# synsense/HaghighatshoarMuir2024

Hardware: AMD Instinct MI355X
Metric: audio samples/sec through STHT+RZCC+SNN beamform, 7-mic 48kHz 360-DoA; DoA MAE vs ref (higher is better)
Workload: dtype f64

## Files before the change

### __graft_entry__.py

```python
import os
import subprocess
import sys

ROOT = os.path.dirname(os.path.abspath(__file__))
if ROOT not in sys.path:
    sys.path.insert(0, ROOT)


def build() -> None:
    env = dict(os.environ)
    subprocess.check_call(["make", "-s", "-j4", "-C", os.path.join(ROOT, "haghighatshoarmuir2024_amd", "csrc")], env=env)
    subprocess.check_call(["make", "-s", "-C", os.path.join(ROOT, "oracle"), "_build/libmicloc_oracle.so", "_build/libmicloc_oracle_asan.so"], env=env)
    subprocess.check_call([sys.executable, os.path.join(ROOT, "tools", "dev", "make_variant.py"), "stht_valu", "stht_one_tile", "ws_k4", "ws_sparse_lif"], env=env)
    import haghighatshoarmuir2024_amd
    from haghighatshoarmuir2024_amd import _lib

    lib = _lib.load()
    assert lib.micloc_abi_version() == 1


def smoke() -> None:
    import numpy as np
    import torch

    from haghighatshoarmuir2024_amd.runtime import Plan
    from oracle import oracle as O

    assert torch.cuda.is_available(), "smoke() needs the MI355X"
    torch.cuda.set_device(0)
    fs, M, G, T, B = 48_000, 7, 64, 2400, 4
    rng = np.random.RandomState(0)
    ker = O.stht_kernel(fs, 10e-3)
    b, a = O.bandpass(fs, [1000.0, 2000.0])
    w = O.robust_width(fs, 2000.0)
    tau = 1 / (2 * np.pi * 2000.0)
    nir = O.neuron_kernel(np.arange(T) / fs, [tau, tau])
    W = rng.randn(2 * M, G)
    W /= np.linalg.norm(W, axis=0, keepdims=True)
    t = np.arange(T) / fs
    x = np.sin(2 * np.pi * 1500 * t)[None, :, None] * np.ones((B, 1, M)) + 0.5 * rng.randn(B, T, M)
    plan = Plan(M, ker, b, a, w, True, device="cuda:0")
    plan.set_neuron_kernel(nir)
    plan.set_bf_mat(W)
    out = plan.snn_pipeline(plan.to_device(x), want_spikes=True, want_power=True)
    torch.cuda.synchronize()
    spikes = out["spikes"].cpu().numpy()
    power = out["power"].cpu().numpy()
    argmax = out["argmax"].cpu().numpy()
    for i in range(B):
        ref = O.snn_chain(x[i], ker, b, a, w, True, nir, W, want=("spikes", "power"))
        assert np.array_equal(spikes[i], ref["spikes"]), "spikes differ from the oracle"
        assert np.allclose(power[i], ref["power"], rtol=1e-12, atol=0), "power differs from the oracle"
        assert int(argmax[i]) == ref["argmax"]
    print(f"smoke ok: {B} trials x {T} frames, {int((spikes != 0).sum())} spikes bit-exact, power rel err <= 1e-12")


if __name__ == "__main__":
    cmd = sys.argv[1] if len(sys.argv) > 1 else "build"
    {"build": build, "smoke": smoke}[cmd]()
```

### haghighatshoarmuir2024_amd/csrc/beamform.hip

```cpp
#include "micloc_internal.h"

namespace micloc {

typedef double double4_t __attribute__((ext_vector_type(4)));
typedef double double2_t __attribute__((ext_vector_type(2)));

constexpr int BF_THREADS = BF_WAVES * 64;

typedef unsigned uint2_t __attribute__((ext_vector_type(2)));

__device__ __forceinline__ double row_sum4(double x)
{
    unsigned lo = __double2loint(x), hi = __double2hiint(x);
    uint2_t a = __builtin_amdgcn_permlane16_swap(lo, lo, false, false);
    uint2_t b = __builtin_amdgcn_permlane16_swap(hi, hi, false, false);
    const double s = __hiloint2double(b[0], a[0]) + __hiloint2double(b[1], a[1]);
    lo = __double2loint(s);
    hi = __double2hiint(s);
    a = __builtin_amdgcn_permlane32_swap(lo, lo, false, false);
    b = __builtin_amdgcn_permlane32_swap(hi, hi, false, false);
    return __hiloint2double(b[0], a[0]) + __hiloint2double(b[1], a[1]);
}

__device__ __forceinline__ double row_sum4_pair(double a, double b)
{
    uint2_t lo = __builtin_amdgcn_permlane16_swap(__double2loint(a), __double2loint(b), false, false);
    uint2_t hi = __builtin_amdgcn_permlane16_swap(__double2hiint(a), __double2hiint(b), false, false);
    const double s = __hiloint2double(hi[0], lo[0]) + __hiloint2double(hi[1], lo[1]);
    const unsigned sl = __double2loint(s), sh = __double2hiint(s);
    lo = __builtin_amdgcn_permlane32_swap(sl, sl, false, false);
    hi = __builtin_amdgcn_permlane32_swap(sh, sh, false, false);
    return __hiloint2double(hi[0], lo[0]) + __hiloint2double(hi[1], lo[1]);
}

__device__ __forceinline__ void xcd_chunk_order(int &chunk, int &b)
{
    const int nchunks = gridDim.x, nb = gridDim.y;
    const int L = chunk + nchunks * b;
    const int full = (nb >> 3) << 3;
    if (L < full * nchunks) {
        const int j = L >> 3;
        const int bq = j / nchunks;
        chunk = j - bq * nchunks;
        b = 8 * bq + (L & 7);
    }
}

int beamform_nchunks(int T) { return (T + BF_CHUNK - 1) / BF_CHUNK; }

size_t beamform_partial_bytes(int B, int T, int Gp)
{
    return ((size_t)B * ((T + 255) / 256) * Gp * sizeof(double) + 255) & ~(size_t)255;
}


template <int NG, int TILES, int KM, int KV, bool LEAN = false>
__device__ __forceinline__ void ws_stage2_kv(const double *Vl, const double *__restrict__ Wp, int Gp, int wv, int l, int ntile,
                                             double *__restrict__ pout, int j0 = 0)
{
    if constexpr (NG > 0) {
        const int lc = l & 15;
        const int q = l >> 4;
        constexpr int KVD = KV > 0 ? KV : 1;
        double Wf[NG][KM], Wv[NG][KVD];
#pragma unroll
        for (int j = 0; j < NG; ++j) {
            const double *wp = Wp + 16 * (wv + BF_WAVES * (j0 + j)) + lc;
#pragma unroll
            for (int k = 0; k < KM; ++k) Wf[j][k] = wp[(size_t)(4 * k + q) * Gp];
#pragma unroll
            for (int i = 0; i < KV; ++i) Wv[j][i] = wp[(size_t)(4 * KM + i) * Gp];
        }
        double sq[NG];
#pragma unroll
        for (int j = 0; j < NG; ++j) sq[j] = 0.0;
        auto ldv = [&](int tile, double (&V)[KM]) {
            const double *p = Vl + (size_t)(tile < TILES ? tile : TILES - 1) * 256 + l;
#pragma unroll
            for (int k = 0; k < KM; ++k) V[k] = p[64 * k];
        };
        auto ldvv = [&](int tile, double (&Vv)[KVD][4]) {
            const double *p = Vl + (size_t)tile * 256 + 64 * KM + q;
#pragma unroll
            for (int i = 0; i < KV; ++i)
#pragma unroll
                for (int r = 0; r < 4; ++r) Vv[i][r] = p[16 * i + 4 * r];
        };
        auto tile_step = [&](int tile, const double (&V)[KM]) {
            double Vv[KVD][4];
            if (!LEAN) ldvv(tile, Vv);
            double4_t acc[NG];
#pragma unroll
            for (int j = 0; j < NG; ++j) acc[j] = double4_t{0.0, 0.0, 0.0, 0.0};
#pragma unroll
            for (int k = 0; k < KM; ++k)
#pragma unroll
                for (int j = 0; j < NG; ++j) acc[j] = __builtin_amdgcn_mfma_f64_16x16x4f64(V[k], Wf[j][k], acc[j], 0, 0, 0);
#pragma unroll
            for (int i = 0; i < KV; ++i) {
                if (LEAN) {
                    const double *p = Vl + (size_t)tile * 256 + 64 * KM + q + 16 * i;
#pragma unroll
                    for (int r = 0; r < 4; ++r) Vv[0][r] = p[4 * r];
                }
#pragma unroll
                for (int j = 0; j < NG; ++j)
#pragma unroll
                    for (int r = 0; r < 4; ++r) acc[j][r] = __builtin_fma(Vv[LEAN ? 0 : i][r], Wv[j][i], acc[j][r]);
            }
#pragma unroll
            for (int r = 0; r < 4; ++r)
#pragma unroll
                for (int j = 0; j < NG; ++j) sq[j] = __builtin_fma(acc[j][r], acc[j][r], sq[j]);
        };
        if (LEAN) {
            for (int t = 0; t < ntile; ++t) {
                double V[KM];
                ldv(t, V);
                tile_step(t, V);
            }
        } else {
            double VA[KM], VB[KM];
            if (ntile > 0) ldv(0, VA);
            int t = 0;
            for (; t + 1 < ntile; t += 2) {
                ldv(t + 1, VB);
                tile_step(t, VA);
                ldv(t + 2, VA);
                tile_step(t + 1, VB);
            }
            if (t < ntile) tile_step(t, VA);
        }
#pragma unroll
        for (int j = 0; j < NG; ++j) {
            const double s = row_sum4(sq[j]);
            if (l < 16) pout[16 * (wv + BF_WAVES * (j0 + j)) + l] = s;
        }
    }
}

template <int NG, int TILES, bool PING>
__device__ __forceinline__ void ws_stage2(const double *Vl, const double *__restrict__ Wp, int Gp, int wv, int l,
                                          int ntile, double *__restrict__ pout)
{
    if constexpr (NG > 0) {
        const int lc = l & 15;
        const int q = l >> 4;
        double Wf[NG][4];
#pragma unroll
        for (int j = 0; j < NG; ++j) {
            const double *wp = Wp + 16 * (wv + BF_WAVES * j) + lc;
#pragma unroll
            for (int k = 0; k < 4; ++k) Wf[j][k] = wp[(size_t)(4 * k + q) * Gp];
        }
        double sq[NG];
#pragma unroll
        for (int j = 0; j < NG; ++j) sq[j] = 0.0;

        auto ldv = [&](int tile, double (&V)[4]) {
            const double *p = Vl + (size_t)(tile < TILES ? tile : TILES - 1) * 256 + l;
#pragma unroll
            for (int k = 0; k < 4; ++k) V[k] = p[64 * k];
        };
        auto mm = [&](const double (&V)[4], double4_t (&acc)[NG]) {
#pragma unroll
            for (int j = 0; j < NG; ++j) acc[j] = double4_t{0.0, 0.0, 0.0, 0.0};
#pragma unroll
            for (int k = 0; k < 4; ++k)
#pragma unroll
                for (int j = 0; j < NG; ++j)
                    acc[j] = __builtin_amdgcn_mfma_f64_16x16x4f64(V[k], Wf[j][k], acc[j], 0, 0, 0);
        };
        auto sqr = [&](const double4_t (&acc)[NG]) {
#pragma unroll
            for (int r = 0; r < 4; ++r)
#pragma unroll
                for (int j = 0; j < NG; ++j) sq[j] = __builtin_fma(acc[j][r], acc[j][r], sq[j]);
        };

        if (!PING) {
            double VA[4], VB[4];
            double4_t acc[NG];
            if (ntile > 0) ldv(0, VA);
            int t = 0;
            for (; t + 1 < ntile; t += 2) {
                ldv(t + 1, VB);
                mm(VA, acc);
                sqr(acc);
                ldv(t + 2, VA);
                mm(VB, acc);
                sqr(acc);
            }
            if (t < ntile) {
                mm(VA, acc);
                sqr(acc);
            }
        } else if (ntile > 0) {
            double VA[4], VB[4];
            double4_t accA[NG], accB[NG];
            ldv(0, VA);
            ldv(1, VB);
            mm(VA, accA);
            int t = 0;
            auto pin = [&]() {
                __builtin_amdgcn_sched_group_barrier(0x008, 1, 0);
                __builtin_amdgcn_sched_group_barrier(0x100, 2, 0);
                __builtin_amdgcn_sched_group_barrier(0x008, 4 * NG - 1, 0);
                __builtin_amdgcn_sched_group_barrier(0x002, 4 * NG, 0);
                __builtin_amdgcn_sched_barrier(0);
            };
            __builtin_amdgcn_sched_barrier(0);
            for (; t + 2 < ntile; t += 2) {
                mm(VB, accB);
                ldv(t + 2, VA);
                sqr(accA);
                pin();
                mm(VA, accA);
                ldv(t + 3, VB);
                sqr(accB);
                pin();
            }
            if (t + 1 < ntile) {
                mm(VB, accB);
                sqr(accA);
                pin();
                sqr(accB);
            } else {
                sqr(accA);
            }
        }
#pragma unroll
        for (int j = 0; j < NG; ++j) {
            const double s = row_sum4(sq[j]);
            if (l < 16) pout[16 * (wv + BF_WAVES * j) + l] = s;
        }
    }
}

template <int NG, int TILES>
__device__ __forceinline__ void ws_stage2_y(const double *Vl, const double *__restrict__ Wp, int GT, int G, int wv, int l,
                                            int tid, int ntile, int nrows, double *stg, double *__restrict__ yb,
                                            double *__restrict__ pout)
{
    const int Gp = 16 * GT;
    const int lc = l & 15;
    const int q = l >> 4;
    double Wf[NG][4];
#pragma unroll
    for (int j = 0; j < NG; ++j) {
        const int gt = wv + BF_WAVES * j;
        const double *wp = Wp + 16 * (gt < GT ? gt : GT - 1) + lc;
#pragma unroll
        for (int k = 0; k < 4; ++k) Wf[j][k] = wp[(size_t)(4 * k + q) * Gp];
    }
    double sq[NG];
#pragma unroll
    for (int j = 0; j < NG; ++j) sq[j] = 0.0;
    for (int t = 0; t < ntile; ++t) {
        double V[4];
        const double *p = Vl + (size_t)t * 256 + l;
#pragma unroll
        for (int k = 0; k < 4; ++k) V[k] = p[64 * k];
        double4_t acc[NG];
#pragma unroll
        for (int j = 0; j < NG; ++j) acc[j] = double4_t{0.0, 0.0, 0.0, 0.0};
#pragma unroll
        for (int k = 0; k < 4; ++k)
#pragma unroll
            for (int j = 0; j < NG; ++j) acc[j] = __builtin_amdgcn_mfma_f64_16x16x4f64(V[k], Wf[j][k], acc[j], 0, 0, 0);
#pragma unroll
        for (int r = 0; r < 4; ++r)
#pragma unroll
            for (int j = 0; j < NG; ++j) sq[j] = __builtin_fma(acc[j][r], acc[j][r], sq[j]);
#pragma unroll
        for (int j = 0; j < NG; ++j) {
            const int col = 16 * (wv + BF_WAVES * j) + lc;
            if (col < G) {
#pragma unroll
                for (int r = 0; r < 4; ++r) stg[(q + 4 * r) * G + col] = acc[j][r];
            }
        }
        __syncthreads();
        const int rows = nrows - 16 * t < 16 ? nrows - 16 * t : 16;
        const int n = rows * G;
        double *yo = yb + (size_t)16 * t * G;
#pragma unroll 4
        for (int e = tid; e < n; e += BF_THREADS) yo[e] = stg[e];
        __syncthreads();
    }
#pragma unroll
    for (int j = 0; j < NG; ++j) {
        const double s = row_sum4(sq[j]);
        const int gt = wv + BF_WAVES * j;
        if (pout && l < 16 && gt < GT) pout[16 * gt + l] = s;
    }
}

constexpr int WS_KV_WAVES = 6;
template <int NGW, int NT, bool WANT_Y, int KM, int KV>
__global__ __launch_bounds__(BF_THREADS, WANT_Y ? 2 : (KV ? WS_KV_WAVES : (NT == 2 ? 6 : 4))) void beamform_ws_kernel(
    const int8_t *__restrict__ spikes, const double *__restrict__ ntab_g, int NK, const double *__restrict__ Wp, int GT, int C,
    int T, double *__restrict__ partial, int G, double *__restrict__ y, const int *__restrict__ chunk_range)
{
    extern __shared__ __attribute__((aligned(16))) unsigned char smem[];
    const int Gp = 16 * GT;
    const int tid = threadIdx.x;
    const int wv = __builtin_amdgcn_readfirstlane(tid >> 6);
    const int l = tid & 63;
    const int lc = l & 15;
    const int q = l >> 4;
    int chunk = blockIdx.x, b = blockIdx.y;
    xcd_chunk_order(chunk, b);
    if (chunk_range && (chunk < chunk_range[0] || chunk >= chunk_range[1])) return;
    if (chunk_range) T = chunk_range[6];
    const int nchunks = gridDim.x;
    constexpr int CH = BF_WAVES * NT * 16;
    constexpr int TILES = CH / 16;
    const int cs = chunk * CH;

    const int R = CH + 4 * NK - 16;
    double *S = reinterpret_cast<double *>(smem);
    double *Vl = S;
    double *ntab = S + (R * 16 > TILES * 256 ? R * 16 : TILES * 256);
    const int ntab_len = 4 * NK + 16;

    for (int e = tid; e < ntab_len; e += BF_THREADS) ntab[e] = ntab_g[e];
    {
        const int8_t *sb = spikes + (size_t)b * (chunk_range ? chunk_range[3] : T) * C;
        const int tau0 = cs + 16 - 4 * NK;
        const int c = tid & 15;
        constexpr int RP = BF_THREADS / 16;
        const int rr = tid >> 4;
        if (c >= C) {
            for (int rho = rr; rho < R; rho += RP) S[rho * 16 + c] = 0.0;
        } else if (tau0 >= 0 && tau0 + R <= T) {
            const int8_t *p = sb + (size_t)(tau0 + rr) * C + c;
            double *d = S + rr * 16 + c;
            int rho = rr;
            for (; rho + 5 * RP < R; rho += 6 * RP) {
                int8_t v[6];
#pragma unroll
                for (int i = 0; i < 6; ++i) v[i] = p[(size_t)i * RP * C];
#pragma unroll
                for (int i = 0; i < 6; ++i) d[i * RP * 16] = (double)v[i];
                p += (size_t)6 * RP * C;
                d += 6 * RP * 16;
            }
            for (; rho < R; rho += RP) {
                *d = (double)*p;
                p += (size_t)RP * C;
                d += RP * 16;
            }
        } else {
            for (int r0 = rr; r0 < R; r0 += RP * 6) {
                int8_t v[6];
#pragma unroll
                for (int i = 0; i < 6; ++i) {
                    int tau = tau0 + r0 + RP * i;
                    tau = tau < 0 ? 0 : (tau >= T ? T - 1 : tau);
                    v[i] = sb[(size_t)tau * C + c];
                }
#pragma unroll
                for (int i = 0; i < 6; ++i) {
                    const int rho = r0 + RP * i;
                    const int tau = tau0 + rho;
                    if (rho < R) S[rho * 16 + c] = (tau >= 0 && tau < T) ? (double)v[i] : 0.0;
                }
            }
        }
    }
    __syncthreads();

    const int tb0 = cs + wv * NT * 16;
    const bool active = tb0 < T;
    double4_t vacc[NT];
#pragma unroll
    for (int tt = 0; tt < NT; ++tt) vacc[tt] = double4_t{0.0, 0.0, 0.0, 0.0};
    if (active) {
        const double *sp = S + (size_t)(tb0 - cs + q) * 16 + lc;
        const double *np_ = ntab + (lc - q + 4 * NK - 16 + 15 - 12);
        auto kstep = [&](const double *spk_, const double *nir_, int u) {
            const double bn = nir_[12 - 4 * u];
            double a[NT];
#pragma unroll
            for (int tt = 0; tt < NT; ++tt) a[tt] = spk_[(16 * tt + 4 * u) * 16];
#pragma unroll
            for (int tt = 0; tt < NT; ++tt)
                vacc[tt] = __builtin_amdgcn_mfma_f64_16x16x4f64(a[tt], bn, vacc[tt], 0, 0, 0);
        };
        int ks = 0;
        for (; ks + 4 <= NK; ks += 4) {
#pragma unroll
            for (int u = 0; u < 4; ++u) kstep(sp, np_, u);
            sp += 4 * 4 * 16;
            np_ -= 4 * 4;
        }
        for (; ks < NK; ++ks) {
            kstep(sp, np_, 0);
            sp += 4 * 16;
            np_ -= 4;
        }
    }
    __syncthreads();
    if (active) {
        if (tb0 + NT * 16 > T) {
#pragma unroll
            for (int tt = 0; tt < NT; ++tt) {
                const bool tvalid = (tb0 + 16 * tt + lc) < T;
#pragma unroll
                for (int r = 0; r < 4; ++r) vacc[tt][r] = tvalid ? vacc[tt][r] : 0.0;
            }
        }
#pragma unroll
        for (int tt = 0; tt < NT; ++tt) {
            double *vp = Vl + (size_t)(wv * NT + tt) * 256 + l;
#pragma unroll
            for (int r = 0; r < 4; ++r) vp[64 * r] = vacc[tt][r];
        }
    }
    __syncthreads();

    int ntile = (T - cs + 15) >> 4;
    ntile = ntile > TILES ? TILES : ntile;
    double *pout = partial + ((size_t)b * nchunks + chunk) * Gp;
    if constexpr (WANT_Y) {
        double *stg = ntab + ((ntab_len + 1) & ~1);
        ws_stage2_y<NGW, TILES>(Vl, Wp, GT, G, wv, l, tid, ntile, T - cs, stg, y + ((size_t)b * T + cs) * G,
                                partial ? pout : nullptr);
        return;
    }
    const int wo = wv;
    if constexpr (KM < 4 || NGW == 4) {
        constexpr bool LEAN = (KV > 0 || NGW == 4) && WS_KV_WAVES >= 6;
        if constexpr (LEAN && NGW == 4) {
            ws_stage2_kv<2, TILES, KM, KV, true>(Vl, Wp, Gp, wo, l, ntile, pout, 0);
            if (wo + BF_WAVES * 3 < GT)
                ws_stage2_kv<2, TILES, KM, KV, true>(Vl, Wp, Gp, wo, l, ntile, pout, 2);
            else
                ws_stage2_kv<1, TILES, KM, KV, true>(Vl, Wp, Gp, wo, l, ntile, pout, 2);
            return;
        }
        if (wo + BF_WAVES * (NGW - 1) < GT)
            ws_stage2_kv<NGW, TILES, KM, KV, LEAN>(Vl, Wp, Gp, wo, l, ntile, pout);
        else
            ws_stage2_kv<NGW - 1, TILES, KM, KV, LEAN>(Vl, Wp, Gp, wo, l, ntile, pout);
        return;
    }
    if (wo + BF_WAVES * (NGW - 1) < GT)
        ws_stage2<NGW, TILES, NT != 2>(Vl, Wp, Gp, wo, l, ntile, pout);
    else
        ws_stage2<NGW - 1, TILES, NT != 2>(Vl, Wp, Gp, wo, l, ntile, pout);
}

static size_t ws_lds_bytes(const NeuronTab &nt, int NT, int Gy = 0)
{
    const size_t tile = (size_t)(BF_WAVES * NT * 16 + 4 * nt.NK - 16) * 16, vfrag = (size_t)BF_WAVES * NT * 256;
    const size_t tab = (size_t)(4 * nt.NK + 16);
    return ((tile > vfrag ? tile : vfrag) + (Gy ? ((tab + 1) & ~(size_t)1) + (size_t)16 * Gy : tab)) * sizeof(double);
}

template <int NGW, int NT, bool WANT_Y, int KM = 4, int KV = 0>
static hipError_t launch_ws_n(const BeamformW &W, const NeuronTab &nt, const int8_t *spikes, int B, int T,
                              double *partial, double *y, hipStream_t stream)
{
    if constexpr (!WANT_Y && KM == 4) {
        if (!VARIANT_WS_FOUR_KSTEPS) {
#define WS_K(KM_, KV_) return launch_ws_n<NGW, NT, false, KM_, KV_>(W, nt, spikes, B, T, partial, y, stream)
            switch (W.C) {
                case 1: case 2: case 3: case 4: WS_K(1, 0);
                case 6: WS_K(1, 2);
                case 5: case 7: case 8: WS_K(2, 0);
                case 10: WS_K(2, 2);
                case 9: case 11: case 12: WS_K(3, 0);
                case 14: WS_K(3, 2);
                default: break;
            }
#undef WS_K
        }
    }
    dim3 grid((T + BF_WAVES * NT * 16 - 1) / (BF_WAVES * NT * 16), B), block(BF_THREADS);
    const size_t lds = ws_lds_bytes(nt, NT, WANT_Y ? W.G : 0);
    if (lds > 160 * 1024) return hipErrorInvalidValue;
    auto k = &beamform_ws_kernel<NGW, NT, WANT_Y, KM, KV>;
    hipError_t e = hipFuncSetAttribute(reinterpret_cast<const void *>(k), hipFuncAttributeMaxDynamicSharedMemorySize,
                                       160 * 1024);
    if (e != hipSuccess) return e;
    hipLaunchKernelGGL(k, grid, block, lds, stream, spikes, nt.tab, nt.NK, W.Wp, W.GT, W.C, T, partial, W.G, y, W.chunk_range);
    return hipGetLastError();
}

constexpr int WS_NT = 2;

static bool ws_eligible(const BeamformW &W, const NeuronTab &nt, bool want_y)
{
    return W.CT == 1 && W.GT <= 4 * BF_WAVES && ws_lds_bytes(nt, WS_NT, want_y ? W.G : 0) <= 160 * 1024;
}

template <int NT, bool WANT_Y>
static hipError_t launch_ws_nt(const BeamformW &W, const NeuronTab &nt, const int8_t *spikes, int B, int T,
                               double *partial, double *y, hipStream_t stream)
{
    switch ((W.GT + BF_WAVES - 1) / BF_WAVES) {
        case 1: return launch_ws_n<1, NT, WANT_Y>(W, nt, spikes, B, T, partial, y, stream);
        case 2: return launch_ws_n<2, NT, WANT_Y>(W, nt, spikes, B, T, partial, y, stream);
        case 3: return launch_ws_n<3, NT, WANT_Y>(W, nt, spikes, B, T, partial, y, stream);
        case 4: return launch_ws_n<4, NT, WANT_Y>(W, nt, spikes, B, T, partial, y, stream);
        default: return hipErrorInvalidValue;
    }
}

static hipError_t launch_ws(const BeamformW &W, const NeuronTab &nt, const int8_t *spikes, int B, int T,
                            double *partial, double *y, hipStream_t stream, int *nchunks)
{
    *nchunks = (T + BF_WAVES * WS_NT * 16 - 1) / (BF_WAVES * WS_NT * 16);
    if (y) return launch_ws_nt<WS_NT, true>(W, nt, spikes, B, T, partial, y, stream);
    return launch_ws_nt<WS_NT, false>(W, nt, spikes, B, T, partial, nullptr, stream);
}

template <int TILES, int KM, int KV, bool FLAT>
__device__ __forceinline__ void wsc_stage2_y(const double *Vl, const double *__restrict__ Wp, int GT, int Gc, int wv, int l, int ntile,
                                             int nrows, double2 *stg, double2 *__restrict__ yb, double *__restrict__ pout)
{
    const int Gp = 16 * GT, GTc = GT >> 1;
    const int lc = l & 15, q = l >> 4;
    constexpr int KVD = KV > 0 ? KV : 1;
    for (int p0 = 0; 16 * p0 < GTc; ++p0) {
        const int g0 = 256 * p0;
        const int ncol = Gc - g0 < 256 ? Gc - g0 : 256;
        double Wf[2][2][KM], Wv[2][2][KVD];
        bool own[2];
#pragma unroll
        for (int j = 0; j < 2; ++j) {
            const int ct = 16 * p0 + wv + BF_WAVES * j;
            own[j] = ct < GTc;
#pragma unroll
            for (int part = 0; part < 2; ++part) {
                const double *wp = Wp + 16 * ((own[j] ? ct : GTc - 1) + part * GTc) + lc;
#pragma unroll
                for (int k = 0; k < KM; ++k) Wf[j][part][k] = wp[(size_t)(4 * k + q) * Gp];
#pragma unroll
                for (int i = 0; i < KV; ++i) Wv[j][part][i] = wp[(size_t)(4 * KM + i) * Gp];
            }
        }
        double sq[2][2] = {{0.0, 0.0}, {0.0, 0.0}};
        for (int t = 0; t < ntile; ++t) {
            double V[KM];
            const double *p = Vl + (size_t)t * 256 + l;
#pragma unroll
            for (int k = 0; k < KM; ++k) V[k] = p[64 * k];
            double4_t acc[2][2];
#pragma unroll
            for (int j = 0; j < 2; ++j)
#pragma unroll
                for (int part = 0; part < 2; ++part) acc[j][part] = double4_t{0.0, 0.0, 0.0, 0.0};
#pragma unroll
            for (int k = 0; k < KM; ++k)
#pragma unroll
                for (int j = 0; j < 2; ++j)
#pragma unroll
                    for (int part = 0; part < 2; ++part)
                        acc[j][part] = __builtin_amdgcn_mfma_f64_16x16x4f64(V[k], Wf[j][part][k], acc[j][part], 0, 0, 0);
#pragma unroll
            for (int i = 0; i < KV; ++i) {
                double Vv[4];
                const double *pv = Vl + (size_t)t * 256 + 64 * KM + q + 16 * i;
#pragma unroll
                for (int r = 0; r < 4; ++r) Vv[r] = pv[4 * r];
#pragma unroll
                for (int j = 0; j < 2; ++j)
#pragma unroll
                    for (int part = 0; part < 2; ++part)
#pragma unroll
                        for (int r = 0; r < 4; ++r) acc[j][part][r] = __builtin_fma(Vv[r], Wv[j][part][i], acc[j][part][r]);
            }
#pragma unroll
            for (int r = 0; r < 4; ++r)
#pragma unroll
                for (int j = 0; j < 2; ++j)
#pragma unroll
                    for (int part = 0; part < 2; ++part) sq[j][part] = __builtin_fma(acc[j][part][r], acc[j][part][r], sq[j][part]);
#pragma unroll
            for (int h = 0; h < 2; ++h) {
#pragma unroll
                for (int j = 0; j < 2; ++j) {
                    const int col = 16 * (wv + BF_WAVES * j) + lc;
                    if (own[j] && col < ncol) {
#pragma unroll
                        for (int rr = 0; rr < 2; ++rr) {
                            double2 v;
                            v.x = acc[j][0][2 * h + rr];
                            v.y = acc[j][1][2 * h + rr];
                            stg[(q + 4 * rr) * ncol + col] = v;
                        }
                    }
                }
                __syncthreads();
                if constexpr (FLAT) {
                    const int r0 = 16 * t + 8 * h;
                    const int n = (nrows - r0 < 8 ? (nrows - r0 > 0 ? nrows - r0 : 0) : 8) * Gc;
                    double2 *yo = yb + (size_t)r0 * Gc;
                    for (int e = wv * 64 + l; e < n; e += BF_THREADS) yo[e] = stg[e];
                } else {
                    const int trow = 16 * t + 8 * h + wv;
                    if (trow < nrows) {
                        double2 *yo = yb + (size_t)trow * Gc + g0;
                        const double2 *so = stg + wv * ncol;
                        for (int c = l; c < ncol; c += 64) yo[c] = so[c];
                    }
                }
                __syncthreads();
            }
        }
#pragma unroll
        for (int j = 0; j < 2; ++j)
#pragma unroll
            for (int part = 0; part < 2; ++part) {
                const double s = row_sum4(sq[j][part]);
                const int ct = 16 * p0 + wv + BF_WAVES * j;
                if (pout && l < 16 && own[j]) pout[16 * (ct + part * GTc) + l] = s;
            }
    }
}

template <int KM, int KV, bool WANT_Y, bool FLAT = false>
__global__ __launch_bounds__(BF_THREADS, WANT_Y ? 4 : 6) void beamform_wsc_kernel(const double *__restrict__ pre,
                                                                                   const double *__restrict__ Wp, int GT, int C, int T,
                                                                                   int Ts, double *__restrict__ partial, int Gc,
                                                                                   double *__restrict__ y)
{
    extern __shared__ __attribute__((aligned(16))) unsigned char smem[];
    constexpr int NT = 2;
    constexpr int CH = BF_WAVES * NT * 16;
    constexpr int TILES = CH / 16;
    constexpr int KF = KM + (KV > 0 ? 1 : 0);
    const int Gp = 16 * GT;
    const int tid = threadIdx.x;
    const int wv = __builtin_amdgcn_readfirstlane(tid >> 6);
    const int l = tid & 63;
    const int lc = l & 15;
    const int q = l >> 4;
    const int chunk = blockIdx.x, b = blockIdx.y;
    const int nchunks = gridDim.x;
    const int cs = chunk * CH;
    double *Vl = reinterpret_cast<double *>(smem);

    {
        const double *pb = pre + (size_t)b * C * Ts;
        double v[NT][KF];
#pragma unroll
        for (int tt = 0; tt < NT; ++tt) {
            const int t = cs + (wv * NT + tt) * 16 + lc;
#pragma unroll
            for (int k = 0; k < KF; ++k) {
                const int c = 4 * k + q;
                v[tt][k] = pb[(size_t)(c < C ? c : C - 1) * Ts + (t < T ? t : T - 1)];
            }
        }
#pragma unroll
        for (int tt = 0; tt < NT; ++tt) {
            const int t = cs + (wv * NT + tt) * 16 + lc;
#pragma unroll
            for (int k = 0; k < KF; ++k) {
                const int c = 4 * k + q;
                Vl[(size_t)(wv * NT + tt) * 256 + 64 * k + l] = (t < T && c < C) ? v[tt][k] : 0.0;
            }
        }
    }
    __syncthreads();

    int ntile = (T - cs + 15) >> 4;
    ntile = ntile > TILES ? TILES : ntile;
    double *pout = partial ? partial + ((size_t)b * nchunks + chunk) * Gp : nullptr;
    if constexpr (WANT_Y) {
        double2 *stg = reinterpret_cast<double2 *>(Vl + TILES * 256);
        wsc_stage2_y<TILES, KM, KV, FLAT>(Vl, Wp, GT, Gc, wv, l, ntile, T - cs, stg, reinterpret_cast<double2 *>(y) + ((size_t)b * T + cs) * Gc,
                                    pout);
    } else {
        const int ntl = (GT - wv + BF_WAVES - 1) / BF_WAVES;
        for (int j0 = 0; j0 < ntl; j0 += 3) {
            const int n = ntl - j0;
            if (n >= 3)
                ws_stage2_kv<3, TILES, KM, KV, true>(Vl, Wp, Gp, wv, l, ntile, pout, j0);
            else if (n == 2)
                ws_stage2_kv<2, TILES, KM, KV, true>(Vl, Wp, Gp, wv, l, ntile, pout, j0);
            else
                ws_stage2_kv<1, TILES, KM, KV, true>(Vl, Wp, Gp, wv, l, ntile, pout, j0);
        }
    }
}

constexpr int WSC_CHUNK = BF_WAVES * 2 * 16;

static bool wsc_eligible(const BeamformW &W) { return W.CT == 1 && W.complex_pairs && (W.GT & 1) == 0; }

template <int KM, int KV>
static hipError_t launch_wsc_k(const BeamformW &W, const double *pre, int B, int T, int Ts, double *y, double *partial,
                               hipStream_t stream)
{
    const size_t lds = (size_t)16 * 256 * sizeof(double) + (y ? (size_t)8 * 256 * sizeof(double2) : 0);
    dim3 grid((T + WSC_CHUNK - 1) / WSC_CHUNK, B), block(BF_THREADS);
    if (y && W.G / 2 <= 256)
        hipLaunchKernelGGL((beamform_wsc_kernel<KM, KV, true, true>), grid, block, lds, stream, pre, W.Wp, W.GT, W.C, T, Ts, partial, W.G / 2, y);
    else if (y)
        hipLaunchKernelGGL((beamform_wsc_kernel<KM, KV, true>), grid, block, lds, stream, pre, W.Wp, W.GT, W.C, T, Ts, partial, W.G / 2, y);
    else
        hipLaunchKernelGGL((beamform_wsc_kernel<KM, KV, false>), grid, block, lds, stream, pre, W.Wp, W.GT, W.C, T, Ts, partial, W.G / 2, y);
    return hipGetLastError();
}

static hipError_t launch_wsc(const BeamformW &W, const double *pre, int B, int T, int Ts, double *y, double *partial, hipStream_t stream)
{
#define WSC_K(KM_, KV_) return launch_wsc_k<KM_, KV_>(W, pre, B, T, Ts, y, partial, stream)
    switch (W.C) {
        case 2: case 4: WSC_K(1, 0);
        case 6: WSC_K(1, 2);
        case 8: WSC_K(2, 0);
        case 10: WSC_K(2, 2);
        case 12: WSC_K(3, 0);
        case 14: WSC_K(3, 2);
        case 16: WSC_K(4, 0);
        default: return hipErrorInvalidValue;
    }
#undef WSC_K
}

constexpr int GEN_COLS = 32;
constexpr int gen_nt(int CT) { return CT > 4 ? 1 : 2; }
constexpr int gen_nsub(int CT) { return CT > 4 ? 4 : 1; }
constexpr int gen_chunk(int CT) { return BF_WAVES * gen_nt(CT) * 16 * gen_nsub(CT); }

int beamform_nchunks_ct(int T, int CT)
{
    const int ch = CT > 4 ? gen_chunk(8) : gen_chunk(1);
    return (T + ch - 1) / ch;
}

struct GenLds {
    size_t u_doubles, total_bytes;
};
static GenLds gen_lds(int CT, int NK, bool src_spikes, int Gp)
{
    const int Kp = 16 * CT, NT = gen_nt(CT), NSUB = gen_nsub(CT);
    size_t u = (size_t)Kp * GEN_COLS;
    if (src_spikes) {
        const size_t tile = (size_t)(4 * NK + 16) + ((size_t)(BF_WAVES * NT * 16 + 4 * NK - 16) * Kp + 7) / 8;
        u = tile > u ? tile : u;
    }
    u = (u + 1) & ~(size_t)1;
    size_t d = (size_t)Kp * GEN_COLS + u + (size_t)2 * BF_WAVES * GEN_COLS + (NSUB > 1 ? (size_t)Gp + GEN_COLS : 0);
    return {u, d * sizeof(double)};
}

template <int CT, bool SRC_SPIKES, bool WANT_Y>
__global__ __launch_bounds__(BF_THREADS, 4) void beamform_gen_kernel(const int8_t *__restrict__ spikes, const double *__restrict__ pre,
                                                                      const double *__restrict__ ntab_g, int NK,
                                                                      const double *__restrict__ Wp, int GT, int C, int G, int T, int Ts,
                                                                      double *__restrict__ y, int y_complex, double *__restrict__ partial,
                                                                      const int *__restrict__ chunk_range, int u_doubles, int vec_stage)
{
    extern __shared__ __attribute__((aligned(16))) unsigned char smem[];
    constexpr int NT = gen_nt(CT), NSUB = gen_nsub(CT);
// ... 543 lines not shown
```

Before: 3.617 billion.

## Add persistent walking beamform kernel that reuses spike halo across consecutive chunks

Adds a persistent-style LIF+beamform kernel in which each workgroup walks a contiguous range of (batch, chunk) items instead of handling one chunk. The halo rows from the previous chunk are carried in LDS, and the next chunk's spikes are prefetched into registers while the current chunk computes. Beamform weights are loaded into registers once per workgroup. This is meant to cut redundant halo loads, per-chunk weight loads and launch-grid overhead, at the cost of extra synchronisation, more registers and a more complex partition. The previous one-chunk path stays as a fallback and as a build variant.

```diff
diff --git a/__graft_entry__.py b/__graft_entry__.py
--- a/__graft_entry__.py
+++ b/__graft_entry__.py
@@ -11,7 +11,7 @@
     env = dict(os.environ)
     subprocess.check_call(["make", "-s", "-j4", "-C", os.path.join(ROOT, "haghighatshoarmuir2024_amd", "csrc")], env=env)
     subprocess.check_call(["make", "-s", "-C", os.path.join(ROOT, "oracle"), "_build/libmicloc_oracle.so", "_build/libmicloc_oracle_asan.so"], env=env)
-    subprocess.check_call([sys.executable, os.path.join(ROOT, "tools", "dev", "make_variant.py"), "stht_valu", "stht_one_tile", "ws_k4", "ws_sparse_lif"], env=env)
+    subprocess.check_call([sys.executable, os.path.join(ROOT, "tools", "dev", "make_variant.py"), "stht_valu", "stht_one_tile", "ws_k4", "ws_sparse_lif", "ws_one_chunk"], env=env)
     import haghighatshoarmuir2024_amd
     from haghighatshoarmuir2024_amd import _lib
 
diff --git a/haghighatshoarmuir2024_amd/csrc/beamform_walk.hip b/haghighatshoarmuir2024_amd/csrc/beamform_walk.hip
--- /dev/null
+++ b/haghighatshoarmuir2024_amd/csrc/beamform_walk.hip
@@ -0,0 +1,329 @@
+#include "micloc_internal.h"
+#include "ws_partition.h"
+
+namespace micloc {
+
+typedef double double4_t __attribute__((ext_vector_type(4)));
+typedef double double2_t __attribute__((ext_vector_type(2)));
+typedef unsigned uint2_t __attribute__((ext_vector_type(2)));
+
+constexpr int BF_THREADS = BF_WAVES * 64;
+constexpr int WS_NT = 2;
+
+hipError_t launch_lif_beamform_one_chunk(const BeamformW &W, const NeuronTab &nt, const int8_t *spikes, int B, int T, double *y,
+                                         double *partial, hipStream_t stream, int *nchunks);
+
+__device__ __forceinline__ double row_sum4(double x)
+{
+    unsigned lo = __double2loint(x), hi = __double2hiint(x);
+    uint2_t a = __builtin_amdgcn_permlane16_swap(lo, lo, false, false);
+    uint2_t b = __builtin_amdgcn_permlane16_swap(hi, hi, false, false);
+    const double s = __hiloint2double(b[0], a[0]) + __hiloint2double(b[1], a[1]);
+    lo = __double2loint(s);
+    hi = __double2hiint(s);
+    a = __builtin_amdgcn_permlane32_swap(lo, lo, false, false);
+    b = __builtin_amdgcn_permlane32_swap(hi, hi, false, false);
+    return __hiloint2double(b[0], a[0]) + __hiloint2double(b[1], a[1]);
+}
+
+template <int NG, int NT, int KM, int KV, bool LEAN>
+__device__ __forceinline__ void ws_walk_run(unsigned char *smem, const int8_t *__restrict__ spikes, const double *__restrict__ ntab_g,
+                                            int NK, const double *__restrict__ Wp, int Gp, int C, int T, double *__restrict__ partial,
+                                            int nchunks, long long spikes_bytes, int p0, int len, int wv, int tid)
+{
+    constexpr int CH = BF_WAVES * NT * 16, TILES = CH / 16;
+    constexpr int NGD = NG > 0 ? NG : 1, KVD = KV > 0 ? KV : 1;
+    static_assert(BF_THREADS == 2 * CH, "one thread per half row of the new rows");
+    auto fresh_tid = [&]() {
+        int t = tid;
+        asm volatile("" : "+v"(t));
+        return t;
+    };
+    const int HR = 4 * NK - 16;
+    double *S = reinterpret_cast<double *>(smem);
+    double *Vl = S;
+    double *ntab = S + (CH + HR) * 16;
+
+    for (int e = tid; e < 4 * NK + 16; e += BF_THREADS) ntab[e] = ntab_g[e];
+    double Wf[NGD][KM], Wv[NGD][KVD];
+    if constexpr (NG > 0) {
+        const int lc = tid & 15, q = (tid & 63) >> 4;
+#pragma unroll
+        for (int j = 0; j < NG; ++j) {
+            const double *wp = Wp + 16 * (wv + BF_WAVES * j) + lc;
+#pragma unroll
+            for (int k = 0; k < KM; ++k) Wf[j][k] = wp[(size_t)(4 * k + q) * Gp];
+#pragma unroll
+            for (int i = 0; i < KV; ++i) Wv[j][i] = wp[(size_t)(4 * KM + i) * Gp];
+        }
+    }
+    int b = p0 / nchunks, chunk = p0 - b * nchunks;
+
+    auto half_mask = [](int nb) { return nb >= 8 ? ~0ull : (nb <= 0 ? 0ull : ((1ull << (8 * nb)) - 1)); };
+    const unsigned long long cmask0 = half_mask(C), cmask1 = half_mask(C - 8);
+    auto load_new = [&](int b_, int chunk_) -> unsigned long long {
+        const int t = fresh_tid();
+        const int nr = t >> 1, nh = t & 1;
+        const int voff = nr * C + 8 * nh;
+        const long long cb = ((long long)b_ * T + (long long)chunk_ * CH) * C;
+        const long long rem = spikes_bytes - cb;
+        const int remi = rem > (1 << 20) ? (1 << 20) : (int)rem;
+        unsigned long long w = 0;
+        if (nr < T - chunk_ * CH) {
+            const int8_t *p = spikes + cb + voff;
+            if (voff + 8 <= remi) {
+                __builtin_memcpy(&w, p, 8);
+            } else {
+                for (int c = 0; c < 8 && voff + c < remi; ++c) w |= (unsigned long long)(uint8_t)p[c] << (8 * c);
+            }
+        }
+        return w;
+    };
+    auto store_new = [&](unsigned long long w) {
+        const int t = fresh_tid();
+        const int nr = t >> 1, nh = t & 1;
+        w &= nh ? cmask1 : cmask0;
+        const unsigned lo = (unsigned)w, hi = (unsigned)(w >> 32);
+        double2_t *d = reinterpret_cast<double2_t *>(S + (HR + nr) * 16 + 8 * nh);
+        d[0] = double2_t{(double)(int8_t)(lo), (double)(int8_t)(lo >> 8)};
+        d[1] = double2_t{(double)(int8_t)(lo >> 16), (double)(int8_t)(lo >> 24)};
+        d[2] = double2_t{(double)(int8_t)(hi), (double)(int8_t)(hi >> 8)};
+        d[3] = double2_t{(double)(int8_t)(hi >> 16), (double)(int8_t)(hi >> 24)};
+    };
+
+    unsigned long long wnew = load_new(b, chunk);
+    {
+        const int8_t *sb = spikes + (size_t)b * T * C;
+        const int tau0 = chunk * CH - HR;
+        const int c = tid & 15;
+        for (int rho = tid >> 4; rho < HR; rho += BF_THREADS / 16) {
+            const int tau = tau0 + rho;
+            S[rho * 16 + c] = (c < C && tau >= 0) ? (double)sb[(size_t)tau * C + c] : 0.0;
+        }
+    }
+
+    const int rel = wv * NT * 16;
+    for (int it = 0;; ++it) {
+        const int cs = chunk * CH;
+        store_new(wnew);
+        __syncthreads();
+
+        const int tb0 = cs + rel;
+        const bool active = tb0 < T;
+        double4_t vacc[NT];
+#pragma unroll
+        for (int tt = 0; tt < NT; ++tt) vacc[tt] = double4_t{0.0, 0.0, 0.0, 0.0};
+        if (active) {
+            const int t = fresh_tid();
+            const int lc = t & 15, q = (t & 63) >> 4;
+            const double *sp = S + (size_t)(rel + q) * 16 + lc;
+            const double *np_ = ntab + (lc - q + 4 * NK - 16 + 15 - 12);
+            auto kstep = [&](const double *spk_, const double *nir_, int u) {
+                const double bn = nir_[12 - 4 * u];
+                double a[NT];
+#pragma unroll
+                for (int tt = 0; tt < NT; ++tt) a[tt] = spk_[(16 * tt + 4 * u) * 16];
+#pragma unroll
+                for (int tt = 0; tt < NT; ++tt) vacc[tt] = __builtin_amdgcn_mfma_f64_16x16x4f64(a[tt], bn, vacc[tt], 0, 0, 0);
+            };
+            int ks = 0;
+            for (; ks + 4 <= NK; ks += 4) {
+#pragma unroll
+                for (int u = 0; u < 4; ++u) kstep(sp, np_, u);
+                sp += 4 * 4 * 16;
+                np_ -= 4 * 4;
+            }
+            for (; ks < NK; ++ks) {
+                kstep(sp, np_, 0);
+                sp += 4 * 16;
+                np_ -= 4;
+            }
+        }
+        __syncthreads();
+        if (active) {
+            const int l = fresh_tid() & 63, lc = l & 15;
+            if (tb0 + NT * 16 > T) {
+#pragma unroll
+                for (int tt = 0; tt < NT; ++tt) {
+                    const bool tvalid = (tb0 + 16 * tt + lc) < T;
+#pragma unroll
+                    for (int r = 0; r < 4; ++r) vacc[tt][r] = tvalid ? vacc[tt][r] : 0.0;
+                }
+            }
+#pragma unroll
+            for (int tt = 0; tt < NT; ++tt) {
+                double *vp = Vl + (size_t)(wv * NT + tt) * 256 + l;
+#pragma unroll
+                for (int r = 0; r < 4; ++r) vp[64 * r] = vacc[tt][r];
+            }
+        }
+        const bool more = it + 1 < len;
+        int nb_ = b, nchunk = chunk + 1;
+        if (nchunk == nchunks) {
+            nchunk = 0;
+            ++nb_;
+        }
+        if (more) wnew = load_new(nb_, nchunk);
+        __syncthreads();
+
+        if constexpr (NG > 0) {
+            const int l = fresh_tid() & 63, q = l >> 4;
+            int ntile = (T - cs + 15) >> 4;
+            ntile = ntile > TILES ? TILES : ntile;
+            double sq[NG];
+#pragma unroll
+            for (int j = 0; j < NG; ++j) sq[j] = 0.0;
+            auto ldv = [&](int tile, double (&V)[KM]) {
+                const double *p = Vl + (size_t)(tile < TILES ? tile : TILES - 1) * 256 + l;
+#pragma unroll
+                for (int k = 0; k < KM; ++k) V[k] = p[64 * k];
+            };
+            auto tile_step = [&](int tile, const double (&V)[KM]) {
+                double Vv[KVD][4];
+                if (!LEAN) {
+                    const double *p = Vl + (size_t)tile * 256 + 64 * KM + q;
+#pragma unroll
+                    for (int i = 0; i < KV; ++i)
+#pragma unroll
+                        for (int r = 0; r < 4; ++r) Vv[i][r] = p[16 * i + 4 * r];
+                }
+                double4_t acc[NG];
+#pragma unroll
+                for (int j = 0; j < NG; ++j) acc[j] = double4_t{0.0, 0.0, 0.0, 0.0};
+#pragma unroll
+                for (int k = 0; k < KM; ++k)
+#pragma unroll
+                    for (int j = 0; j < NG; ++j) acc[j] = __builtin_amdgcn_mfma_f64_16x16x4f64(V[k], Wf[j][k], acc[j], 0, 0, 0);
+#pragma unroll
+                for (int i = 0; i < KV; ++i) {
+                    if (LEAN) {
+                        const double *p = Vl + (size_t)tile * 256 + 64 * KM + q + 16 * i;
+#pragma unroll
+                        for (int r = 0; r < 4; ++r) Vv[0][r] = p[4 * r];
+                    }
+#pragma unroll
+                    for (int j = 0; j < NG; ++j)
+#pragma unroll
+                        for (int r = 0; r < 4; ++r) acc[j][r] = __builtin_fma(Vv[LEAN ? 0 : i][r], Wv[j][i], acc[j][r]);
+                }
+#pragma unroll
+                for (int r = 0; r < 4; ++r)
+#pragma unroll
+                    for (int j = 0; j < NG; ++j) sq[j] = __builtin_fma(acc[j][r], acc[j][r], sq[j]);
+            };
+            if (LEAN) {
+                for (int t = 0; t < ntile; ++t) {
+                    double V[KM];
+                    ldv(t, V);
+                    tile_step(t, V);
+                }
+            } else {
+                double VA[KM], VB[KM];
+                if (ntile > 0) ldv(0, VA);
+                int t = 0;
+                for (; t + 1 < ntile; t += 2) {
+                    ldv(t + 1, VB);
+                    tile_step(t, VA);
+                    ldv(t + 2, VA);
+                    tile_step(t + 1, VB);
+                }
+                if (t < ntile) tile_step(t, VA);
+            }
+            double *pout = partial + ((size_t)b * nchunks + chunk) * Gp;
+#pragma unroll
+            for (int j = 0; j < NG; ++j) {
+                const double s = row_sum4(sq[j]);
+                if (l < 16) pout[16 * (wv + BF_WAVES * j) + l] = s;
+            }
+        }
+        if (!more) break;
+
+        const int ts = fresh_tid();
+        double2_t hc = double2_t{0.0, 0.0};
+        if (ts < HR * 8 && nchunk != 0) hc = *reinterpret_cast<const double2_t *>(S + CH * 16 + 2 * ts);
+        __syncthreads();
+        if (ts < HR * 8) *reinterpret_cast<double2_t *>(S + 2 * ts) = hc;
+        b = nb_;
+        chunk = nchunk;
+    }
+}
+
+template <int NGW, int NT, int KM, int KV>
+__global__ __launch_bounds__(BF_THREADS, 6) void beamform_ws_walk_kernel(const int8_t *__restrict__ spikes, const double *__restrict__ ntab_g,
+                                                                         int NK, const double *__restrict__ Wp, int GT, int C, int T,
+                                                                         double *__restrict__ partial, int nchunks, long long spikes_bytes,
+                                                                         WsPartition part)
+{
+    extern __shared__ __attribute__((aligned(16))) unsigned char smem[];
+    const int tid = threadIdx.x;
+    const int wv = __builtin_amdgcn_readfirstlane(tid >> 6);
+    const int w = xcd_walk(blockIdx.x, gridDim.x);
+    long long first;
+    int len;
+    ws_partition_run(part, w, first, len);
+    constexpr bool LEAN = KV > 0 || (KM == 4 && NGW == 3);
+    if (wv + BF_WAVES * (NGW - 1) < GT)
+        ws_walk_run<NGW, NT, KM, KV, LEAN>(smem, spikes, ntab_g, NK, Wp, 16 * GT, C, T, partial, nchunks, spikes_bytes, (int)first, len, wv, tid);
+    else
+        ws_walk_run<NGW - 1, NT, KM, KV, LEAN>(smem, spikes, ntab_g, NK, Wp, 16 * GT, C, T, partial, nchunks, spikes_bytes, (int)first, len, wv, tid);
+}
+
+template <int NGW, int KM, int KV>
+static hipError_t launch_walk_k(const BeamformW &W, const NeuronTab &nt, const int8_t *spikes, int B, int T, double *partial, size_t lds,
+                                hipStream_t stream)
+{
+    static int num_cu = 0;
+    if (num_cu == 0) {
+        int dev = 0;
+        hipDeviceProp_t prop;
+        if (hipGetDevice(&dev) != hipSuccess || hipGetDeviceProperties(&prop, dev) != hipSuccess) return hipErrorInvalidDevice;
+        num_cu = prop.multiProcessorCount > 0 ? prop.multiProcessorCount : 256;
+    }
+    const int nchunks = (T + BF_WAVES * WS_NT * 16 - 1) / (BF_WAVES * WS_NT * 16);
+    const WsPartition part = ws_partition((long long)nchunks * B, 3 * num_cu);
+    auto kw = &beamform_ws_walk_kernel<NGW, WS_NT, KM, KV>;
+    hipLaunchKernelGGL(kw, dim3(part.nwg), dim3(BF_THREADS), lds, stream, spikes, nt.tab, nt.NK, W.Wp, W.GT, W.C, T, partial, nchunks,
+                       (long long)B * T * W.C, part);
+    return hipGetLastError();
+}
+
+template <int NGW>
+static hipError_t launch_walk_n(const BeamformW &W, const NeuronTab &nt, const int8_t *spikes, int B, int T, double *partial, size_t lds,
+                                hipStream_t stream)
+{
+#define WS_K(KM_, KV_) return launch_walk_k<NGW, KM_, KV_>(W, nt, spikes, B, T, partial, lds, stream)
+    if (!VARIANT_WS_FOUR_KSTEPS) {
+        switch (W.C) {
+            case 1: case 2: case 3: case 4: WS_K(1, 0);
+            case 6: WS_K(1, 2);
+            case 5: case 7: case 8: WS_K(2, 0);
+            case 10: WS_K(2, 2);
+            case 9: case 11: case 12: WS_K(3, 0);
+            case 14: WS_K(3, 2);
+            default: break;
+        }
+    }
+    WS_K(4, 0);
+#undef WS_K
+}
+
+hipError_t launch_lif_beamform(const BeamformW &W, const NeuronTab &nt, const int8_t *spikes, int B, int T, double *y, double *partial,
+                               hipStream_t stream, int *nchunks)
+{
+    const int HR = 4 * nt.NK - 16;
+    const int nch = (T + BF_WAVES * WS_NT * 16 - 1) / (BF_WAVES * WS_NT * 16);
+    const size_t lds = ((size_t)(BF_WAVES * WS_NT * 16 + HR) * 16 + 4 * nt.NK + 16) * sizeof(double);
+    const long long items = (long long)nch * B;
+    if (!VARIANT_WS_ONE_CHUNK && partial && !y && !W.chunk_range && W.CT == 1 && W.C >= 1 && W.C <= 16 && W.GT >= 1 && W.GT <= 3 * BF_WAVES &&
+        HR >= 0 && HR <= 64 && B >= 1 && T >= 1 && items < (1ll << 31)) {
+        *nchunks = nch;
+        switch ((W.GT + BF_WAVES - 1) / BF_WAVES) {
+            case 1: return launch_walk_n<1>(W, nt, spikes, B, T, partial, lds, stream);
+            case 2: return launch_walk_n<2>(W, nt, spikes, B, T, partial, lds, stream);
+            default: return launch_walk_n<3>(W, nt, spikes, B, T, partial, lds, stream);
+        }
+    }
+    return launch_lif_beamform_one_chunk(W, nt, spikes, B, T, y, partial, stream, nchunks);
+}
+
+}
diff --git a/haghighatshoarmuir2024_amd/csrc/ws_partition.h b/haghighatshoarmuir2024_amd/csrc/ws_partition.h
--- /dev/null
+++ b/haghighatshoarmuir2024_amd/csrc/ws_partition.h
@@ -0,0 +1,35 @@
+#pragma once
+
+#if defined(__HIPCC__) || defined(__CUDACC__)
+#define WS_PART_HD __host__ __device__
+#else
+#define WS_PART_HD
+#endif
+
+namespace micloc {
+
+constexpr bool VARIANT_WS_ONE_CHUNK = false;
+
+struct WsPartition {
+    int nwg;
+    int base;
+    int extra;
+};
+
+WS_PART_HD inline WsPartition ws_partition(long long items, int slots)
+{
+    WsPartition p;
+    if (slots < 1) slots = 1;
+    p.nwg = items < (long long)slots ? (int)items : slots;
+    p.base = p.nwg > 0 ? (int)(items / p.nwg) : 0;
+    p.extra = p.nwg > 0 ? (int)(items - (long long)p.base * p.nwg) : 0;
+    return p;
+}
+
+WS_PART_HD inline void ws_partition_run(const WsPartition &p, int w, long long &first, int &len)
+{
+    first = (long long)w * p.base + (w < p.extra ? w : p.extra);
+    len = p.base + (w < p.extra ? 1 : 0);
+}
+
+}
```

Result: slower. 3.522 billion (-2.6%).

## Balance stage-2 beamform work across waves when group tiles divide unevenly

Applied to the files above, without the earlier changes.

Adds a balanced stage-2 path for the KV variants with 2 or 3 groups per wave. It applies when the number of group tiles leaves a remainder that splits evenly among the light waves. Light waves compute partial sums of squares for the heavy waves' extra group over an initial range of tiles and hand them over through a small new LDS buffer, so the heavy waves need fewer tiles at the end. This targets tail imbalance in which some waves do one more group than the others. In exchange it adds LDS per block, a __syncthreads, and reloads weights per pass.

```diff
diff --git a/haghighatshoarmuir2024_amd/csrc/beamform.hip b/haghighatshoarmuir2024_amd/csrc/beamform.hip
--- a/haghighatshoarmuir2024_amd/csrc/beamform.hip
+++ b/haghighatshoarmuir2024_amd/csrc/beamform.hip
@@ -296,6 +296,105 @@
     }
 }
 
+constexpr int WS_HAND_DOUBLES = (BF_WAVES - 1) * 64;
+constexpr bool VARIANT_WS_UNBALANCED = false;
+
+__host__ __device__ constexpr bool ws_balanced_grid(int GT)
+{
+    const int h = GT & (BF_WAVES - 1);
+    return h != 0 && h % (BF_WAVES - h) == 0;
+}
+
+template <int NG, int KM, int KV>
+__device__ __forceinline__ void ws_bal_tiles(const double *Vl, const double (&Wf)[NG][KM], const double (&Wv)[NG][KV], double (&sq)[NG],
+                                             int l, int t0, int t1)
+{
+    const int q = l >> 4;
+    for (int t = t0; t < t1; ++t) {
+        const double *p = Vl + (size_t)t * 256 + l;
+        double V[KM];
+#pragma unroll
+        for (int k = 0; k < KM; ++k) V[k] = p[64 * k];
+        double4_t acc[NG];
+#pragma unroll
+        for (int j = 0; j < NG; ++j) acc[j] = double4_t{0.0, 0.0, 0.0, 0.0};
+#pragma unroll
+        for (int k = 0; k < KM; ++k)
+#pragma unroll
+            for (int j = 0; j < NG; ++j) acc[j] = __builtin_amdgcn_mfma_f64_16x16x4f64(V[k], Wf[j][k], acc[j], 0, 0, 0);
+#pragma unroll
+        for (int i = 0; i < KV; ++i) {
+            const double *pv = Vl + (size_t)t * 256 + 64 * KM + q + 16 * i;
+            double Vv[4];
+#pragma unroll
+            for (int r = 0; r < 4; ++r) Vv[r] = pv[4 * r];
+#pragma unroll
+            for (int j = 0; j < NG; ++j)
+#pragma unroll
+                for (int r = 0; r < 4; ++r) acc[j][r] = __builtin_fma(Vv[r], Wv[j][i], acc[j][r]);
+        }
+#pragma unroll
+        for (int r = 0; r < 4; ++r)
+#pragma unroll
+            for (int j = 0; j < NG; ++j) sq[j] = __builtin_fma(acc[j][r], acc[j][r], sq[j]);
+    }
+}
+
+template <int NG, int KM, int KV>
+__device__ __forceinline__ void ws_bal_load(const double *__restrict__ Wp, int Gp, int gt0, int l, double (&Wf)[NG][KM], double (&Wv)[NG][KV])
+{
+#pragma unroll
+    for (int j = 0; j < NG; ++j) {
+        const double *wp = Wp + 16 * (gt0 + BF_WAVES * j) + (l & 15);
+#pragma unroll
+        for (int k = 0; k < KM; ++k) Wf[j][k] = wp[(size_t)(4 * k + (l >> 4)) * Gp];
+#pragma unroll
+        for (int i = 0; i < KV; ++i) Wv[j][i] = wp[(size_t)(4 * KM + i) * Gp];
+    }
+}
+
+template <int NGW, int KM, int KV>
+__device__ __forceinline__ void ws_stage2_balanced(const double *Vl, const double *__restrict__ Wp, int Gp, int GT, int wv, int l,
+                                                   int ntile, double *__restrict__ pout, double *hand)
+{
+    constexpr int NB = NGW - 1;
+    const int h = GT & (BF_WAVES - 1), k = h / (BF_WAVES - h);
+    const int s = ntile / (k + 1);
+    int a = ntile - (2 * k * s + NB) / (2 * NB);
+    a = a < 0 ? 0 : a;
+    const bool heavy = wv < h;
+    double Wf1[1][KM], Wv1[1][KV], sq1[1];
+    if (!heavy && s > 0) {
+        for (int c = 0; c < k; ++c) {
+            const int w = (wv - h) * k + c;
+            ws_bal_load<1, KM, KV>(Wp, Gp, w + BF_WAVES * NB, l, Wf1, Wv1);
+            sq1[0] = 0.0;
+            ws_bal_tiles<1, KM, KV>(Vl, Wf1, Wv1, sq1, l, 0, s);
+            hand[w * 64 + l] = sq1[0];
+        }
+    }
+    const int ta = heavy ? ntile : a;
+    double Wf[NB][KM], Wv[NB][KV], sq[NB];
+    ws_bal_load<NB, KM, KV>(Wp, Gp, wv, l, Wf, Wv);
+#pragma unroll
+    for (int j = 0; j < NB; ++j) sq[j] = 0.0;
+    ws_bal_tiles<NB, KM, KV>(Vl, Wf, Wv, sq, l, 0, ta);
+    __syncthreads();
+    ws_bal_tiles<NB, KM, KV>(Vl, Wf, Wv, sq, l, ta, ntile);
+#pragma unroll
+    for (int j = 0; j < NB; ++j) {
+        const double r = row_sum4(sq[j]);
+        if (l < 16) pout[16 * (wv + BF_WAVES * j) + l] = r;
+    }
+    if (heavy) {
+        ws_bal_load<1, KM, KV>(Wp, Gp, wv + BF_WAVES * NB, l, Wf1, Wv1);
+        sq1[0] = s > 0 ? hand[wv * 64 + l] : 0.0;
+        ws_bal_tiles<1, KM, KV>(Vl, Wf1, Wv1, sq1, l, s, ntile);
+        const double r = row_sum4(sq1[0]);
+        if (l < 16) pout[16 * (wv + BF_WAVES * NB) + l] = r;
+    }
+}
+
 constexpr int WS_KV_WAVES = 6;
 template <int NGW, int NT, bool WANT_Y, int KM, int KV>
 __global__ __launch_bounds__(BF_THREADS, WANT_Y ? 2 : (KV ? WS_KV_WAVES : (NT == 2 ? 6 : 4))) void beamform_ws_kernel(
@@ -440,6 +539,12 @@
                 ws_stage2_kv<1, TILES, KM, KV, true>(Vl, Wp, Gp, wo, l, ntile, pout, 2);
             return;
         }
+        if constexpr (LEAN && KV > 0 && (NGW == 2 || NGW == 3) && !WANT_Y && !VARIANT_WS_UNBALANCED) {
+            if (!chunk_range && ws_balanced_grid(GT)) {
+                ws_stage2_balanced<NGW, KM, KV>(Vl, Wp, Gp, GT, wo, l, ntile, pout, ntab + ((ntab_len + 1) & ~1));
+                return;
+            }
+        }
         if (wo + BF_WAVES * (NGW - 1) < GT)
             ws_stage2_kv<NGW, TILES, KM, KV, LEAN>(Vl, Wp, Gp, wo, l, ntile, pout);
         else
@@ -456,7 +561,8 @@
 {
     const size_t tile = (size_t)(BF_WAVES * NT * 16 + 4 * nt.NK - 16) * 16, vfrag = (size_t)BF_WAVES * NT * 256;
     const size_t tab = (size_t)(4 * nt.NK + 16);
-    return ((tile > vfrag ? tile : vfrag) + (Gy ? ((tab + 1) & ~(size_t)1) + (size_t)16 * Gy : tab)) * sizeof(double);
+    const size_t hand = VARIANT_WS_UNBALANCED ? 0 : ((tab + 1) & ~(size_t)1) - tab + WS_HAND_DOUBLES;
+    return ((tile > vfrag ? tile : vfrag) + (Gy ? ((tab + 1) & ~(size_t)1) + (size_t)16 * Gy : tab + hand)) * sizeof(double);
 }
 
 template <int NGW, int NT, bool WANT_Y, int KM = 4, int KV = 0>
```

Result: slower. 3.592 billion before, 3.511 billion after (-2.2%).
